# Rita-zi/WavTokenizer

Measured on AMD Instinct MI355X. Metric: audio-seconds/sec encode+decode, 24 kHz 3 s clips, higher is better.
Workload: dtype f32 (split-f16 x3 products)

## Files before the change

include/wavtokenizer_amd.h:

```cpp
#ifndef WAVTOKENIZER_AMD_H
#define WAVTOKENIZER_AMD_H

#include <stddef.h>
#include <stdint.h>

#ifdef __cplusplus
extern "C" {
#endif

typedef enum {
    WT_OK = 0,
    WT_ERR_INVALID = -1,
    WT_ERR_MISSING_TENSOR = -2,
    WT_ERR_SHAPE = -3,
    WT_ERR_HIP = -4,
    WT_ERR_NOT_INITED = -5,
    WT_ERR_RANGE = -6,
    WT_ERR_LSTM_SYNC = -7,
    WT_ERR_INDEX = -8
} wt_status;

enum wt_status_bits {
    WT_STATUS_BIT_LSTM = 1,
    WT_STATUS_BIT_RANGE = 2,
// ... 144 lines not shown
    const float* A2;
    const float* B;
    const float* bias;
    const float* R;
    const float* gamma;
    float* C;
    float* C2;
    uint32_t* status;
} wt_gemm_desc;
typedef struct {
    int32_t BM, BN, waves_m, waves_n, stages, ks, prod, staged, bias_cache, G, tiles;
} wt_launch_form;
size_t wt_gemm_probe_workspace_bytes(const wt_gemm_desc* d);
int wt_gemm_probe(const wt_gemm_desc* d, wt_launch_form* form, void* workspace, void* stream);

enum { WT_OP_GN_APPLY = 0, WT_OP_GN_STATS = 1, WT_OP_ROWNORM = 2, WT_OP_SOFTMAX = 3, WT_OP_ISTFT_OLA = 4, WT_OP_CONV_FIRST = 5,
       WT_OP_CONV_LAST = 6, WT_OP_TRANSPOSE = 7, WT_OP_CONVTR = 8, WT_OP_ROW_SUMSQ = 9, WT_OP_S32_AMAX = 10 };
enum { WT_OPK_GN_TILE = 1, WT_OPK_GN_CHUNK = 2, WT_OPK_GN_STATS = 3, WT_OPK_ROWNORM = 4, WT_OPK_DWCONV_LN = 5,
       WT_OPK_SOFTMAX_REG = 6, WT_OPK_SOFTMAX_RMW = 7, WT_OPK_ISTFT_OLA = 8, WT_OPK_CONV_FIRST = 9, WT_OPK_CONV_LAST32 = 10,
       WT_OPK_CONV_LAST = 11, WT_OPK_TRANSPOSE = 12, WT_OPK_CONVTR = 13, WT_OPK_ROW_SUMSQ = 14, WT_OPK_S32_AMAX = 15,
       WT_OPK_TRANSPOSE_MIXED = 16, WT_OPK_GN_MIXED = 17, WT_OPK_DWCONV_LN_MIXED = 18, WT_OPK_SOFTMAX_REG_MIXED = 19,
       WT_OPK_SOFTMAX_RMW_MIXED = 20, WT_OPK_ISTFT_OLA_MIXED = 21 };
typedef struct {
    int32_t size;
    int32_t op;
    int32_t B, L, C;
    int32_t groups, mode, flag, out_s32;
    int32_t ld, k, stride, Cout, n_fft, hop, Kq;
    float eps;
    int64_t n;
// ... 42 lines not shown
```

wavtokenizer_amd/_capi.py:

```python
from __future__ import annotations

import ctypes
import os
from ctypes import POINTER, c_char_p, c_float, c_int32, c_int64, c_size_t, c_void_p

_HERE = os.path.dirname(os.path.abspath(__file__))
LIB_PATH = os.environ.get("WAVTOK_HIP_LIB") or os.path.join(_HERE, "libwavtok_hip.so")

EXPORTS = [
    "wt_last_error", "wt_version", "wt_model_create", "wt_model_destroy", "wt_model_export_bytes", "wt_model_export", "wt_packed_info", "wt_packed_verify", "wt_packed_bytes",
    "wt_model_create_packed", "wt_model_hop", "wt_model_weight_bytes",
    "wt_plan_create", "wt_plan_create_ex", "wt_plan_range_sites", "wt_plan_range_report", "wt_model_persistent_lstm", "wt_device_info", "wt_plan_destroy", "wt_plan_workspace_bytes", "wt_plan_frames", "wt_plan_num_launches", "wt_plan_graph_replays",
    "wt_plan_find_buffer", "wt_plan_buffer_info", "wt_plan_buffer_name", "wt_plan_status", "wt_plan_num_steps", "wt_plan_step_name",
    "wt_plan_set_timing", "wt_plan_read_timing", "wt_model_split_ok", "wt_model_status", "wt_model_take_bad_codes", "wt_encode", "wt_codes_to_features",
    "wt_decode", "wt_seanet_decode", "wt_head", "wt_unit_run", "wt_sconv1d", "wt_linear", "wt_conv1d_s32", "wt_vq_workspace_bytes",
    "wt_vq_nearest", "wt_vq_nearest_f32", "wt_resblock", "wt_resblock_down", "wt_gemm_probe_workspace_bytes", "wt_gemm_probe", "wt_op_probe",
    "wt_resampler_create", "wt_resampler_destroy", "wt_resampler_out_length", "wt_convert_audio", "wt_pcm16",
    "wt_linear_overlap_add", "wt_encode_mixed", "wt_plan_min_clip_length", "wt_sconv_geometry", "wt_decode_mixed",
]

WT_PLAN_ENCODE, WT_PLAN_DECODE, WT_PLAN_SEANET_DECODER, WT_PLAN_HEAD, WT_PLAN_UNIT_LSTM = 0, 1, 2, 3, 4
WT_PLAN_DECODE_MIXED = 5
WT_PLAN_FLAG_KEEP_STAGES = 1
WT_PLAN_FLAG_FP32_GEMM = 2
WT_PLAN_FLAG_STEP_LSTM = 4
WT_PLAN_FLAG_GRAPH = 8
WT_PLAN_FLAG_UNFUSED = 16
WT_PLAN_FLAG_RANGE_REPORT = 32
WT_PLAN_FLAG_MIXED_LENGTH = 64
WT_SITE_ENCODER, WT_SITE_BB_EMBED, WT_SITE_RES0, WT_SITE_RES1, WT_SITE_ATTN, WT_SITE_RES2, WT_SITE_RES3 = 0, 1, 2, 3, 4, 5, 6
WT_SITE_CNX0, WT_SITE_HEAD, WT_SITE_SEANET_DECODER = 7, 40, 41
# ... 11 lines not shown


class WtTensor(ctypes.Structure):
    _fields_ = [("name", c_char_p), ("data", POINTER(c_float)), ("numel", c_int64)]


class WtGemmDesc(ctypes.Structure):
    _fields_ = ([("size", c_int32), ("engine", c_int32), ("epi", c_int32), ("out", c_int32), ("pro", c_int32), ("b_is_act", c_int32),
                 ("M", c_int32), ("N", c_int32), ("K", c_int32)]
                + [(n, c_int32) for n in ("T_in", "T_out", "Cin", "taps", "stride", "dil", "pad_left", "pad_mode", "Tp",
                                         "K1", "nz", "tap_pair", "head_kb")]
                + [("alpha", c_float)]
                + [(n, c_int64) for n in ("a_bstride", "a_rstride", "a2_bstride", "a2_rstride", "w_rstride", "c_rstride",
                                         "r_rstride", "zA", "zW", "zC")]
                + [(n, c_void_p) for n in ("A", "A2", "B", "bias", "R", "gamma", "C", "C2", "status")])


class WtLaunchForm(ctypes.Structure):
    _fields_ = [(n, c_int32) for n in ("BM", "BN", "waves_m", "waves_n", "stages", "ks", "prod", "staged", "bias_cache", "G", "tiles")]


WT_OP_GN_APPLY, WT_OP_GN_STATS, WT_OP_ROWNORM, WT_OP_SOFTMAX, WT_OP_ISTFT_OLA, WT_OP_CONV_FIRST = 0, 1, 2, 3, 4, 5
WT_OP_CONV_LAST, WT_OP_TRANSPOSE, WT_OP_CONVTR, WT_OP_ROW_SUMSQ, WT_OP_S32_AMAX = 6, 7, 8, 9, 10
WT_OPK_NAMES = {1: "gn_tile", 2: "gn_chunk", 3: "gn_stats", 4: "rownorm", 5: "dwconv_ln", 6: "softmax_reg", 7: "softmax_rmw",
                8: "istft_ola", 9: "conv_first", 10: "conv_last32", 11: "conv_last", 12: "transpose", 13: "convtr",
                14: "row_sumsq", 15: "s32_amax", 16: "transpose_mixed", 17: "gn_mixed", 18: "dwconv_ln_mixed",
                19: "softmax_reg_mixed", 20: "softmax_rmw_mixed", 21: "istft_ola_mixed"}


class WtOpDesc(ctypes.Structure):
# ... 86 lines not shown
    lib.wt_head.argtypes = [c_void_p, c_void_p, c_void_p, c_void_p, c_void_p]
    lib.wt_sconv1d.argtypes = [c_void_p, c_void_p, c_void_p, c_void_p, c_int32, c_int64, c_int32, c_int32, c_int32,
                               c_int32, c_int32, c_int32, c_void_p]
    lib.wt_linear.argtypes = [c_void_p, c_void_p, c_void_p, c_void_p, c_int64, c_int32, c_int32, c_int32, c_void_p, c_void_p]
    lib.wt_conv1d_s32.argtypes = [c_void_p, c_void_p, c_void_p, c_void_p, c_int32, c_int64, c_int32, c_int32, c_int32,
                                  c_int32, c_int32, c_void_p, c_void_p]
    lib.wt_vq_workspace_bytes.argtypes = [c_int64, c_int32, c_int32]
    lib.wt_vq_workspace_bytes.restype = c_size_t
    lib.wt_vq_nearest.argtypes = [c_void_p, c_void_p, c_int64, c_int32, c_int32, c_void_p, c_void_p, c_void_p]
    lib.wt_vq_nearest_f32.argtypes = [c_void_p, c_void_p, c_int64, c_int32, c_int32, c_void_p, c_void_p, c_void_p]
    lib.wt_resblock.argtypes = [c_void_p] * 11 + [c_int32, c_int64, c_int32, c_int32, c_int32, c_int32, c_void_p]
    lib.wt_resblock_down.argtypes = [c_void_p] * 12 + [c_int32, c_int64, c_int32, c_void_p]
    lib.wt_gemm_probe_workspace_bytes.argtypes = [POINTER(WtGemmDesc)]
    lib.wt_gemm_probe_workspace_bytes.restype = c_size_t
    lib.wt_gemm_probe.argtypes = [POINTER(WtGemmDesc), POINTER(WtLaunchForm), c_void_p, c_void_p]
    lib.wt_op_probe.argtypes = [POINTER(WtOpDesc), POINTER(WtOpForm), c_void_p]
    lib.wt_resampler_create.argtypes = [c_int32, c_int32, c_int32, POINTER(c_void_p)]
    lib.wt_resampler_destroy.argtypes = [c_void_p]
    lib.wt_resampler_destroy.restype = None
    lib.wt_resampler_out_length.argtypes = [c_void_p, c_int64]
    lib.wt_resampler_out_length.restype = c_int64
    lib.wt_convert_audio.argtypes = [c_void_p, c_void_p, c_int32, c_int32, c_int64, c_void_p, c_void_p]
    lib.wt_pcm16.argtypes = [c_void_p, c_int64, ctypes.c_float, c_int32, c_void_p, c_void_p, c_void_p]
    lib.wt_linear_overlap_add.argtypes = [c_void_p, c_void_p, c_int32, c_int64, c_int64, c_int64, c_int64, c_void_p, c_void_p]
    return lib


lib = _load()


# ... 5 lines not shown
```

wavtokenizer_amd/csrc/common.h:

```cpp
#pragma once
#include <hip/hip_runtime.h>
#include <stdint.h>
#include <stdio.h>
#include <stdlib.h>
#include <mutex>
#include <string>

namespace wt {

void set_error(const std::string& msg);

#define WT_HIP_CHECK(expr)                                                                      \
    do {                                                                                        \
        hipError_t _e = (expr);                                                                 \
        if (_e != hipSuccess) {                                                                 \
            ::wt::set_error(std::string(#expr) + ": " + hipGetErrorString(_e));                 \
            return -4;                                                                          \
        }                                                                                       \
    } while (0)

struct PerDeviceOnce {
    std::mutex mu;
    bool seen[64] = {};
    template <class F> int run(F&& f) {
// ... 178 lines not shown
    int stage_off = 0;
    int pc_off = 0;
    float acc_scale = 1.f;
    const float* acc_scale_dev = nullptr;
    unsigned* status = nullptr;
    unsigned long long* dbg_stamps = nullptr;
    LaunchForm* form = nullptr;
};

int gemm_vq_parts(int N);
int check_gemm(const GemmArgs& a, int pro, int epi);
int check_gemm16s(const GemmArgs& a, int epi, int out, const int* mix_geom = nullptr);
int launch_gemm(const GemmArgs& a, int pro, int epi, hipStream_t s);
int launch_gemm16s(const GemmArgs& a, int epi, int out, hipStream_t s, const int* mix_geom = nullptr);
int gemm16s_vq_parts(int N);
int launch_split_s32(const float* x, void* out, long n, hipStream_t s, const float* scale_dev = nullptr);
int launch_unsplit_s32(const void* s32, float* out, long n, float inv_scale, hipStream_t s);
int launch_pow2_scales(const float* a, long na, const float* b, long nb, unsigned* bits2, float* out3, hipStream_t s);

int launch_conv_first(const float* wav, const float* w , const float* bias, float* y, int B, long T,
                      int k, int Cout, hipStream_t s);
int launch_conv_last(const float* x , const float* w , const float* bias, float* y ,
                     int B, long T, int Cin, int k, int elu_in, hipStream_t s);
int launch_transpose(const float* in, float* out, int B, int R, int C, hipStream_t s, int out_s32 = 0, const int* lens = nullptr);
size_t gn_part_floats(int B, int L, int groups);
int launch_gn_stats(const float* x, const float* gamma, const float* beta, float* scale, float* shift, int B, int L,
                    int C, int groups, float eps, hipStream_t s, float* part = nullptr, const int* lens = nullptr);
int launch_gn_apply(const float* x, const float* gamma, const float* beta, float* scale, float* shift, float* y,
                    int swish, int B, int L, int C, int groups, float eps, hipStream_t s, int out_s32 = 0, float* part = nullptr,
                    const int* lens = nullptr);
// ... 93 lines not shown
```

wavtokenizer_amd/csrc/gemm16s.hip:

```cpp
#include "common.h"

#include <cmath>
#include <stdlib.h>
#include <type_traits>

namespace wt {

typedef float f32x4 __attribute__((ext_vector_type(4)));
typedef float f32x16 __attribute__((ext_vector_type(16)));
typedef _Float16 f16x8 __attribute__((ext_vector_type(8)));
typedef __attribute__((address_space(3))) void* lds_ptr_t;
static constexpr int SBK = 32;

__device__ __forceinline__ int xcd_remap_s(int orig, int nwg) {
    int q = nwg >> 3, r = nwg & 7;
    int xcd = orig & 7, idx = orig >> 3;
    int base = xcd < r ? xcd * (q + 1) : r * (q + 1) + (xcd - r) * q;
    return base + idx;
}
__device__ __forceinline__ float elu_s(float x) { return elu_med3(x); }
__device__ __forceinline__ float erf_s(float a) {
    const float t = fabsf(a), s = a * a;
    float r = fmaf(-1.72853470e-5f, t, 3.83197126e-4f);
    const float u = fmaf(-3.88396438e-3f, t, 2.42546219e-2f);
// ... 162 lines not shown
#endif
#define G16_NAME gemm16s_kernel
#define G16_PARAMS
#define G16_MIX 0
#include "gemm16s_kernel.inc"
#undef G16_NAME
#undef G16_PARAMS
#undef G16_MIX
#define G16_NAME gemm16s_mixed_kernel
#define G16_PARAMS , const int* __restrict__ mix_geom
#define G16_MIX 1
#include "gemm16s_kernel.inc"
#undef G16_NAME
#undef G16_PARAMS
#undef G16_MIX

__global__ __launch_bounds__(256) void split_s32_kernel(const float* __restrict__ x, _Float16* __restrict__ out, long n,
                                                        const float* __restrict__ scale, unsigned* status) {
    const float sc = scale ? scale[0] : 1.f;
    float amax = 0.f;
    for (long i = (long)blockIdx.x * blockDim.x + threadIdx.x; i < n; i += (long)gridDim.x * blockDim.x) {
        const float v = x[i] * sc;
        amax = amax1(amax, v);
        const _Float16 h = (_Float16)v;
        const long g = (i >> 5) * 64 + (i & 31);
        out[g] = h;
        out[g + 32] = (_Float16)((v - (float)h) * 2048.f);
    }
    range_report(status, amax);
}
// ... 281 lines not shown
    a.group_m = tiles_n192 > 8 ? 8 : 1;
    if (tiles_n192 >= 12 && tiles_n192 % 6 == 0 && a.nz == 1) { a.group_m = 5; a.group_n = 6; }
    if (const char* e = lab_env("WT_GEMM16S_GM")) { a.group_m = atoi(e) > 0 ? atoi(e) : a.group_m; a.group_n = 0; }
    if (const char* e = lab_env("WT_GEMM16S_GN")) a.group_n = atoi(e);
    if (mix_geom) {
#define WT_CASE16S(E, O) if (epi == E && out == O) return launch16s_mixed<E, O>(a, s, mix_geom);
        WT_GEMM16S_MIXED_PAIRS(WT_CASE16S)
#undef WT_CASE16S
    }
#define WT_CASE16S(E, O) if (epi == E && out == O) return launch16s_tiled<E, O>(a, s);
    WT_GEMM16S_PAIRS(WT_CASE16S)
#undef WT_CASE16S
    set_error("gemm16s: unsupported epilogue / output-format pair");
    return -1;
}
#endif

}
```

wavtokenizer_amd/csrc/plan.cpp:

```cpp
#include "model.h"

namespace wt {

static bool site_fp32(const wt_plan* P, int site) { return (P->fp32_sites >> site) & 1u; }
static bool plan_fp32(const wt_plan* P) {
    if ((P->flags & WT_PLAN_FLAG_FP32_GEMM) || !P->model->s32_ok) return true;
    if (P->whole_site == SITE_SEADEC && !P->model->sd_s32_ok) return true;
    return P->whole_site >= 0 && site_fp32(P, P->whole_site);
}
static bool plan_unfused(const wt_plan* P) { return P->flags & WT_PLAN_FLAG_UNFUSED; }
static bool plan_s32(const wt_plan* P) { return !plan_unfused(P) && !plan_fp32(P); }

static int gemm_auto(const wt_plan* P, const GemmArgs& a, int pro, int epi, hipStream_t s) {
    if (P->model->f32_stale.load()) if (int rc = ensure_f32_weights(P->model)) return rc;
    return launch_gemm(a, pro, epi, s);
}

static void set_s32(GemmArgs& a, const S32Copy& c) {
    a.W_hi = c.p; a.acc_scale = c.acc_scale; a.tap_pair = c.tap_pair ? 1 : 0;
}

static int gemm_s32(const GemmArgs& a, int epi, int out, hipStream_t s, const int* mix = nullptr) {
    if (!a.W_hi) { set_error("internal: no S32 copy of this weight"); return WT_ERR_INVALID; }
    return launch_gemm16s(a, epi, out, s, mix);
// ... 155 lines not shown
        if (int rc = launch_fill_u32(s, 0u, (st_numel * sizeof(float) + 15) / 16 * 16, c.stream)) return rc;
        LstmArgs la;
        la.f16x3 = plan_fp32(P) ? 0 : 1;
        la.xg0 = P->ptr(c, xg); la.W0 = la.f16x3 ? w.W0h : w.W0; la.W1 = la.f16x3 ? w.W1h : w.W1; la.b1 = w.b1;
        la.h0 = s; la.h1 = s + (size_t)2 * H * Bp; la.c0 = s + (size_t)4 * H * Bp; la.c1 = la.c0 + (size_t)B * H;
        la.x = P->ptr(c, xin); la.y = P->ptr(c, y); la.B = B; la.L = L; la.H = H; la.elu_out = elu_out ? 1 : 0;
        la.out_s32 = y_s32 ? 1 : 0;
        for (int t = 0; t <= L; ++t)
            if (int rc = launch_lstm_step(la, t, c.stream)) return rc;
        return 0;
    }, L + 2);
    return y;
}

static int plan_resblock_s32(wt_plan* P, const ConvW& c3, const ConvW& sc, const ConvW& cat, int B, long T, int x_raw,
                             int x_elu, const std::string& name, long x_off = 0, long x_bstride = 0, int mix_word = -1) {
    if (!cat.s32.p) { set_error("internal: unfused S32 resblock without an S32 shortcut + conv1 weight"); return -1; }
    const int C = sc.cout;
    const int h = P->buf(name + ".h", (size_t)B * T * (C / 2), BUF_S32 | BUF_ELU);
    GemmArgs a3 = sconv_args(c3, B, T, 1, 1);
    GemmBufs b3{x_elu, -1, h};
    b3.x_off = x_off; b3.mix_word = mix_word >= 0 ? mix_word + GEOM_C3 : -1;
    if (x_bstride) a3.a_bstride = x_bstride;
    gemm_step(P, true, a3, b3, PRO_NONE, EPI_BIAS_ELU, OUT_S32);
    const int o = P->buf(name, (size_t)B * T * C, BUF_S32 | BUF_ELU);
    GemmArgs ac = sconv_args(sc, B, T, 1, 1);
    ac.W = cat.w; ac.w_rstride = cat.cin; ac.bias = cat.b; ac.K = cat.cin; ac.Cin = cat.cin;
    set_s32(ac, cat.s32);
    ac.K1 = C; ac.a2_bstride = T * (C / 2); ac.a2_rstride = C / 2;
    if (x_bstride) ac.a_bstride = x_bstride;
    GemmBufs bc{x_raw, h, o};
    bc.x_off = x_off; bc.mix_word = mix_word >= 0 ? mix_word + GEOM_SC : -1;
    gemm_step(P, true, ac, bc, PRO_NONE, EPI_BIAS_ELU, OUT_S32);
// ... 76 lines not shown
                a.wav = c.in_f; a.e0_w = M->e0_w; a.e0_b = M->e0_b;
                a.W3 = st.c3.w; a.b3 = st.c3.b; a.W1 = st.c1.w; a.b1 = st.c1.b; a.Ws = st.sc.w; a.bs = st.sc.b;
                a.Wd = st.down.w; a.bd = st.down.b; a.y_down = P->ptr(c, y); a.R = st.r;
                a.B = B; a.T = (int)Tc; a.C = st.C;
                return launch_resblock16_down(a, c.stream, geom >= 0 ? &mix : nullptr);
            }, 1, "resblock.fused_down");
            x = y; Tc = ad.T_out; idx += 3;
            continue;
        }
        const std::string name = "enc." + std::to_string(idx);
        const int stage_word = GEOM_STAGE0 + (int)si * GEOM_STAGE_WORDS;
        if (r.fused)
            x = plan_resblock(P, st.c3, st.c1, st.sc, B, Tc, x, name, fuse_elu, (si == 0 && fold_e0) ? M : nullptr, 0, 0, r.s32,
                              mixed ? stage_word + GEOM_C3 : -1);
        else if (r.s32)
            x = plan_resblock_s32(P, st.c3, st.sc, st.cat, B, Tc, x, x_elu, name, 0, 0, mixed ? stage_word : -1);
        else
            x = plan_resblock(P, st.c3, st.c1, st.sc, B, Tc, x, name, fuse_elu);
        if (x < 0) return WT_ERR_INVALID;
        const bool next_s32 = !last && !route[si + 1].fused && route[si + 1].s32;
        const int y = P->buf(out, ynum, next_s32 ? BUF_S32 : BUF_F32);
        const int y2 = (next_s32 || (last && lstm_s32)) ? P->buf(out + ".s32", ynum, BUF_S32 | (next_s32 ? BUF_ELU : 0)) : -1;
        GemmBufs bd{x, -1, y, y2};
        bd.mix_word = mixed ? stage_word + GEOM_DOWN : -1;
        gemm_step(P, r.s32, ad, bd, fuse_elu ? PRO_NONE : PRO_ELU, EPI_BIAS,
                  next_s32 ? OUT_S32_DUAL_ELU : (y2 >= 0 ? OUT_F32_AND_S32 : OUT_F32));
        if (next_s32) x_elu = y2;
        if (last) x_s32 = y2;
        x = y; Tc = ad.T_out; idx += 3;
    }
    const int L = (int)Tc;
// ... 326 lines not shown
```

wavtokenizer_amd/csrc/probe.cpp:

```cpp
#include "model.h"

using namespace wt;

extern "C" {

int wt_codes_to_features(const wt_model* m, const int64_t* codes, int32_t K, int32_t B, int64_t L, float* features,
                         void* stream) {
    if (!m || !codes || !features) { set_error("wt_codes_to_features: null argument"); return WT_ERR_INVALID; }
    if (K < 1 || K > m->arch.num_quantizers) { set_error("wt_codes_to_features: K exceeds the number of codebooks"); return WT_ERR_INVALID; }
    DeviceGuard dg(m->device);
    if (!dg.ok) { set_error("hipSetDevice failed"); return WT_ERR_HIP; }
    return launch_codes_to_features(codes, m->embed.w, K, m->arch.vq_bins, B, L, 512, features, static_cast<hipStream_t>(stream),
                                    m->bad_codes_dev);
}

int wt_sconv1d(const float* x, const float* w, const float* bias, float* y, int32_t B, int64_t T, int32_t Cin,
               int32_t Cout, int32_t k, int32_t stride, int32_t dilation, int32_t elu_input, void* stream) {
    ConvW cw; cw.w = const_cast<float*>(w); cw.b = const_cast<float*>(bias); cw.cout = Cout; cw.cin = Cin; cw.k = k;
    GemmArgs a = sconv_args(cw, B, T, stride, dilation);
    a.A = x; a.C = y;
    return launch_gemm(a, elu_input ? PRO_ELU : PRO_NONE, EPI_BIAS, static_cast<hipStream_t>(stream));
}

static int split_pair(const float* w, long nw, const float* x, long nx, char* ws_w, char* ws_x, char* tail, GemmArgs& a,
// ... 79 lines not shown
    a.w_rstride = d->w_rstride; a.bias = d->bias; a.M = d->M; a.N = d->N; a.K = d->K;
    a.C = d->C; a.c_rstride = d->c_rstride; a.C2 = d->C2; a.R = d->R; a.r_rstride = d->r_rstride; a.gamma = d->gamma;
    a.alpha = d->alpha; a.nz = d->nz; a.zA = d->zA; a.zW = d->zW; a.zC = d->zC; a.head_kb = d->head_kb; a.tap_pair = d->tap_pair ? 1 : 0;
    if (d->engine == 1) {
        a.A = d->A; a.W = d->B;
        return check_gemm(a, d->pro, d->epi) ? WT_ERR_INVALID : WT_OK;
    }
    const ProbeLayout L = probe_layout(*d);
    a.A = reinterpret_cast<const float*>(ws);
    a.A2 = d->A2 ? reinterpret_cast<const float*>(ws + L.oA2) : nullptr;
    a.W = d->B; a.W_hi = ws + L.oB;
    a.status = reinterpret_cast<unsigned*>(d->status);
    return check_gemm16s(a, d->epi, d->out) ? WT_ERR_INVALID : WT_OK;
}

size_t wt_gemm_probe_workspace_bytes(const wt_gemm_desc* d) {
    if (!d || d->size != (int32_t)sizeof(wt_gemm_desc) || d->engine != 0 || d->M <= 0 || d->T_out <= 0 || d->nz < 1) return 0;
    return probe_layout(*d).total;
}

int wt_gemm_probe(const wt_gemm_desc* d, wt_launch_form* form, void* workspace, void* stream) {
    char* ws = static_cast<char*>(workspace);
    GemmArgs a;
    if (int rc = probe_args(d, ws, a)) return rc;
    hipStream_t s = static_cast<hipStream_t>(stream);
    LaunchForm lf;
    a.form = &lf;
    if (d->engine == 1) {
        if (int rc = launch_gemm(a, d->pro, d->epi, s)) return rc;
    } else {
        const ProbeLayout L = probe_layout(*d);
        float* scale_dev = reinterpret_cast<float*>(ws + L.oScale);
        float scale = 1.f;
        if (!d->b_is_act) {
            std::vector<float> h((size_t)L.nB);
            WT_HIP_CHECK(hipMemcpyAsync(h.data(), d->B, (size_t)L.nB * 4, hipMemcpyDeviceToHost, s));
            WT_HIP_CHECK(hipStreamSynchronize(s));
            float amax = 0.f;
            for (long z = 0; z < d->nz; ++z)
                for (long n = 0; n < d->N; ++n)
                    for (long k = 0; k < d->K; ++k) {
                        const float v = std::fabs(h[(size_t)(z * d->zW + n * d->w_rstride + k)]);
                        if (!(v <= 3.0e38f)) { set_error("wt_gemm_probe: a non-finite weight has no S32 copy"); return WT_ERR_INVALID; }
                        amax = std::max(amax, v);
                    }
            scale = s32_weight_scale(amax);
            uint32_t bits;
            memcpy(&bits, &scale, 4);
            if (int rc = launch_fill_u32(scale_dev, bits, 16, s)) return rc;
            a.acc_scale = 1.f / scale;
        }
        if (int rc = launch_split_s32(d->B, ws + L.oB, L.nB, s, scale != 1.f ? scale_dev : nullptr)) return rc;
        if (int rc = launch_split_s32(d->A, ws, L.nA, s)) return rc;
        if (d->A2) if (int rc = launch_split_s32(d->A2, ws + L.oA2, L.nA2, s)) return rc;
        if (int rc = launch_gemm16s(a, d->epi, d->out, s)) return rc;
    }
    if (form) *form = wt_launch_form{lf.BM, lf.BN, lf.waves_m, lf.waves_n, lf.stages, lf.ks, lf.prod, lf.staged, lf.bias_cache, lf.G, lf.tiles};
    return WT_OK;
}

static int op_probe_check(const wt_op_desc* d) {
    auto bad = [](const char* m) { set_error(std::string("wt_op_probe: ") + m); return (int)WT_ERR_INVALID; };
    if (!d || (d->size != (int32_t)sizeof(wt_op_desc) && d->size != (int32_t)offsetof(wt_op_desc, lengths))) return bad("descriptor missing or of another size");
    const int32_t* lengths = d->size == (int32_t)sizeof(wt_op_desc) ? d->lengths : nullptr;
    if (lengths) {
        if (reinterpret_cast<uintptr_t>(lengths) & 3) return bad("lengths misaligned");
        const bool aware = d->op == WT_OP_GN_APPLY || d->op == WT_OP_GN_STATS || (d->op == WT_OP_ROWNORM && d->mode == RN_DWCONV) ||
                           d->op == WT_OP_SOFTMAX || d->op == WT_OP_ISTFT_OLA || d->op == WT_OP_TRANSPOSE;
        if (!aware) return bad("this op has no length-aware launch");
        if (d->op == WT_OP_SOFTMAX && (d->L <= 0 || d->n % d->L)) return bad("the length-aware softmax needs whole clips of L rows");
    }
// ... 188 lines not shown
```

Measured before the change: 38630.

## Fuse resblock k3 conv, ELU and concatenated shortcut GEMM into one chained kernel

Adds a persistent chained GEMM kernel for the S32 resblock. It computes the 3-tap conv, applies bias and ELU, and splits the hidden activation into f16 hi/lo halves held in LDS. The same kernel then runs the concatenated 1x1 and shortcut GEMM, so the hidden tensor never makes a round trip through global memory and one launch is saved per resblock. The kernel holds more LDS and registers and is limited to C of 128 or 256; a probe API is also added for testing.

```diff
diff --git a/include/wavtokenizer_amd.h b/include/wavtokenizer_amd.h
--- a/include/wavtokenizer_amd.h
+++ b/include/wavtokenizer_amd.h
@@ -182,6 +182,22 @@
 size_t wt_gemm_probe_workspace_bytes(const wt_gemm_desc* d);
 int wt_gemm_probe(const wt_gemm_desc* d, wt_launch_form* form, void* workspace, void* stream);
 
+typedef struct {
+    int32_t size;
+    int32_t C, clips, T;
+    int64_t c_rstride;
+    const float* x_elu;
+    const float* x_raw;
+    const float* w3;
+    const float* b3;
+    const float* wcat;
+    const float* bcat;
+    float* out;
+    uint32_t* status;
+} wt_gemm_chain_desc;
+size_t wt_gemm_chain_probe_workspace_bytes(const wt_gemm_chain_desc* d);
+int wt_gemm_chain_probe(const wt_gemm_chain_desc* d, wt_launch_form* form, void* workspace, void* stream);
+
 enum { WT_OP_GN_APPLY = 0, WT_OP_GN_STATS = 1, WT_OP_ROWNORM = 2, WT_OP_SOFTMAX = 3, WT_OP_ISTFT_OLA = 4, WT_OP_CONV_FIRST = 5,
        WT_OP_CONV_LAST = 6, WT_OP_TRANSPOSE = 7, WT_OP_CONVTR = 8, WT_OP_ROW_SUMSQ = 9, WT_OP_S32_AMAX = 10 };
 enum { WT_OPK_GN_TILE = 1, WT_OPK_GN_CHUNK = 2, WT_OPK_GN_STATS = 3, WT_OPK_ROWNORM = 4, WT_OPK_DWCONV_LN = 5,
diff --git a/wavtokenizer_amd/_capi.py b/wavtokenizer_amd/_capi.py
--- a/wavtokenizer_amd/_capi.py
+++ b/wavtokenizer_amd/_capi.py
@@ -15,6 +15,7 @@
     "wt_plan_set_timing", "wt_plan_read_timing", "wt_model_split_ok", "wt_model_status", "wt_model_take_bad_codes", "wt_encode", "wt_codes_to_features",
     "wt_decode", "wt_seanet_decode", "wt_head", "wt_unit_run", "wt_sconv1d", "wt_linear", "wt_conv1d_s32", "wt_vq_workspace_bytes",
     "wt_vq_nearest", "wt_vq_nearest_f32", "wt_resblock", "wt_resblock_down", "wt_gemm_probe_workspace_bytes", "wt_gemm_probe", "wt_op_probe",
+    "wt_gemm_chain_probe_workspace_bytes", "wt_gemm_chain_probe",
     "wt_resampler_create", "wt_resampler_destroy", "wt_resampler_out_length", "wt_convert_audio", "wt_pcm16",
     "wt_linear_overlap_add", "wt_encode_mixed", "wt_plan_min_clip_length", "wt_sconv_geometry", "wt_decode_mixed",
 ]
@@ -56,6 +57,11 @@
                 + [(n, c_int64) for n in ("a_bstride", "a_rstride", "a2_bstride", "a2_rstride", "w_rstride", "c_rstride",
                                          "r_rstride", "zA", "zW", "zC")]
                 + [(n, c_void_p) for n in ("A", "A2", "B", "bias", "R", "gamma", "C", "C2", "status")])
+
+
+class WtGemmChainDesc(ctypes.Structure):
+    _fields_ = ([(n, c_int32) for n in ("size", "C", "clips", "T")] + [("c_rstride", c_int64)]
+                + [(n, c_void_p) for n in ("x_elu", "x_raw", "w3", "b3", "wcat", "bcat", "out", "status")])
 
 
 class WtLaunchForm(ctypes.Structure):
@@ -172,6 +178,9 @@
     lib.wt_gemm_probe_workspace_bytes.argtypes = [POINTER(WtGemmDesc)]
     lib.wt_gemm_probe_workspace_bytes.restype = c_size_t
     lib.wt_gemm_probe.argtypes = [POINTER(WtGemmDesc), POINTER(WtLaunchForm), c_void_p, c_void_p]
+    lib.wt_gemm_chain_probe_workspace_bytes.argtypes = [POINTER(WtGemmChainDesc)]
+    lib.wt_gemm_chain_probe_workspace_bytes.restype = c_size_t
+    lib.wt_gemm_chain_probe.argtypes = [POINTER(WtGemmChainDesc), POINTER(WtLaunchForm), c_void_p, c_void_p]
     lib.wt_op_probe.argtypes = [POINTER(WtOpDesc), POINTER(WtOpForm), c_void_p]
     lib.wt_resampler_create.argtypes = [c_int32, c_int32, c_int32, POINTER(c_void_p)]
     lib.wt_resampler_destroy.argtypes = [c_void_p]
diff --git a/wavtokenizer_amd/csrc/common.h b/wavtokenizer_amd/csrc/common.h
--- a/wavtokenizer_amd/csrc/common.h
+++ b/wavtokenizer_amd/csrc/common.h
@@ -216,6 +216,9 @@
 int launch_gemm(const GemmArgs& a, int pro, int epi, hipStream_t s);
 int launch_gemm16s(const GemmArgs& a, int epi, int out, hipStream_t s, const int* mix_geom = nullptr);
 int gemm16s_vq_parts(int N);
+bool gemm16s_chain_fits(int C);
+int check_gemm16s_chain(const GemmArgs& a3, const GemmArgs& ac);
+int launch_gemm16s_chain(const GemmArgs& a3, const GemmArgs& ac, hipStream_t s);
 int launch_split_s32(const float* x, void* out, long n, hipStream_t s, const float* scale_dev = nullptr);
 int launch_unsplit_s32(const void* s32, float* out, long n, float inv_scale, hipStream_t s);
 int launch_pow2_scales(const float* a, long na, const float* b, long nb, unsigned* bits2, float* out3, hipStream_t s);
diff --git a/wavtokenizer_amd/csrc/gemm16s.hip b/wavtokenizer_amd/csrc/gemm16s.hip
--- a/wavtokenizer_amd/csrc/gemm16s.hip
+++ b/wavtokenizer_amd/csrc/gemm16s.hip
@@ -200,6 +200,317 @@
 #undef G16_NAME
 #undef G16_PARAMS
 #undef G16_MIX
+
+struct ChainArgs {
+    const char* Xe;
+    const char* Xr;
+    long xe_bstride, xe_rstride, xr_bstride, xr_rstride;
+    const char* W3;
+    const char* Wc;
+    long w3_rstride, wc_rstride;
+    const float* b3;
+    const float* bc;
+    float s3, sc;
+    float* C;
+    long c_rstride;
+    int M, T, Tp, pad_left;
+    unsigned* status;
+    unsigned long long* stamp_start;
+    unsigned long long* stamp_end;
+    int res_off, tab_off, bias_off, stage_off;
+};
+
+template <int C, int BM, int WAVES_M, int WAVES_N>
+__global__ __launch_bounds__(64 * WAVES_M * WAVES_N) void gemm16s_chain_kernel(const ChainArgs p) {
+    constexpr int N1 = C / 2, NKC = C / 32, NK1 = 3 * NKC, NKH = N1 / 32, NPASS = C / 128, NK2 = NKC + NKH;
+    constexpr int NS = NK1 + NPASS * NK2;
+    constexpr int NW = WAVES_M * WAVES_N, NT = 64 * NW;
+    constexpr int WM = BM / WAVES_M, WN1 = N1 / WAVES_N, WN2 = 128 / WAVES_N;
+    constexpr int TNH1 = WN1 / 32, TNH2 = WN2 / 32;
+    constexpr int STG = (BM + 128) * 128;
+    constexpr int NPA = BM / 8 / NW, NPB = 128 / 8 / NW, NPT = NPA + NPB;
+    constexpr int NSTAGE = 3;
+    static_assert(NW == 8 && WM == 32 && WN1 == 32 && (WN2 == 32 || WN2 == 64) && (NPASS == 1 || NPASS == 2), "tile forms of C = 128 / 256");
+    static_assert((NKC & (NKC - 1)) == 0 && BM % 64 == 0, "K tiles per tap: a power of two");
+    extern __shared__ __attribute__((aligned(1024))) char smem_s[];
+    constexpr unsigned OOB = 0x80000000u;
+
+    const int tid = threadIdx.x, lane = tid & 63;
+    const int wave = __builtin_amdgcn_readfirstlane(tid >> 6);
+    const int wm = wave / WAVES_N, wn = wave % WAVES_N;
+    const int ntiles = (p.M + BM - 1) / BM, G = gridDim.x;
+    const int nclips = p.M / p.T;
+    if (p.stamp_start && tid == 0)
+        __hip_atomic_fetch_min(p.stamp_start, (unsigned long long)__builtin_amdgcn_s_memrealtime(), __ATOMIC_RELAXED, __HIP_MEMORY_SCOPE_AGENT);
+    auto first_clip = [&](int bm) { return (bm * BM < p.M ? bm * BM : p.M - 1) / p.T; };
+
+    char* const res = smem_s + p.res_off;
+    unsigned* const s_tab = reinterpret_cast<unsigned*>(smem_s + p.tab_off);
+    float* const s_bias = reinterpret_cast<float*>(smem_s + p.bias_off);
+    for (int e = tid; e < N1 + C; e += NT) s_bias[e] = e < N1 ? p.b3[e] : p.bc[e - N1];
+
+    auto build_table = [&](int vb, int par) {
+        if (vb >= ntiles) return;
+        const int bm = xcd_remap_s(vb, ntiles);
+        const int clip0 = first_clip(bm);
+        unsigned* tab = s_tab + par * 4 * BM;
+        for (int e = tid; e < 4 * BM; e += NT) {
+            const int tp = e / BM, r = e - tp * BM;
+            const int m = bm * BM + r;
+            unsigned off = OOB;
+            if (m < p.M) {
+                const int b = m / p.T;
+                const int t = m - b * p.T;
+                if (tp < 3) {
+                    int pos = t - p.pad_left + tp;
+                    pos = pos < 0 ? -pos : pos;
+                    pos = pos >= p.Tp ? 2 * (p.Tp - 1) - pos : pos;
+                    if (pos < p.T) off = (unsigned)(((long)(b - clip0) * p.xe_bstride + (long)pos * p.xe_rstride) * 4);
+                } else {
+                    off = (unsigned)(((long)(b - clip0) * p.xr_bstride + (long)t * p.xr_rstride) * 4);
+                }
+            }
+            tab[e] = off;
+        }
+    };
+
+    const int prow = lane >> 3;
+    int a_row[NPA];
+    unsigned a_chunk[NPA], a_voff[NPA], w3_voff[NPB], wc_voff[NPB];
+#pragma unroll
+    for (int i = 0; i < NPA; ++i) {
+        const int q = wave + NW * i;
+        a_row[i] = q * 8 + prow;
+        a_chunk[i] = (unsigned)(((lane & 7) ^ (((q & 1) << 2) | (lane >> 4))) * 16);
+    }
+#pragma unroll
+    for (int j = 0; j < NPB; ++j) {
+        const int q = BM / 8 + wave + NW * j;
+        const unsigned ch = (unsigned)(((lane & 7) ^ (((q & 1) << 2) | (lane >> 4))) * 16);
+        const int n = (wave + NW * j) * 8 + prow;
+        w3_voff[j] = n < N1 ? (unsigned)((long)n * p.w3_rstride * 4) + ch : OOB;
+        wc_voff[j] = (unsigned)((long)n * p.wc_rstride * 4) + ch;
+    }
+    auto rsrc = [](const char* base, long span) {
+        return __builtin_amdgcn_make_buffer_rsrc(const_cast<char*>(base), 0, (int)(span < 0x7fffffffL ? span : 0x7fffffffL), 0x00020000);
+    };
+    const __amdgpu_buffer_rsrc_t rsW3 = rsrc(p.W3, (long)N1 * p.w3_rstride * 4);
+    const __amdgpu_buffer_rsrc_t rsWc0 = rsrc(p.Wc, 128L * p.wc_rstride * 4);
+    const __amdgpu_buffer_rsrc_t rsWc1 = rsrc(p.Wc + (NPASS - 1) * 128L * p.wc_rstride * 4, 128L * p.wc_rstride * 4);
+    __amdgpu_buffer_rsrc_t rsXe, rsXr;
+    int l_vb = blockIdx.x, l_par = 0, l_step = 0;
+    unsigned l_mask = 0;
+    auto set_arow = [&](int trow) {
+        const unsigned* tab = s_tab + (l_par * 4 + trow) * BM;
+#pragma unroll
+        for (int i = 0; i < NPA; ++i) a_voff[i] = tab[a_row[i]] + a_chunk[i];
+    };
+    auto loader_set_tile = [&](int vb, int par) {
+        l_vb = vb; l_par = par; l_step = 0;
+        if (vb >= ntiles) { l_mask = OOB; return; }
+        const int clip0 = first_clip(xcd_remap_s(vb, ntiles));
+        rsXe = rsrc(p.Xe + (long)clip0 * p.xe_bstride * 4, ((long)(nclips - clip0 - 1) * p.xe_bstride + (long)p.T * p.xe_rstride) * 4);
+        rsXr = rsrc(p.Xr + (long)clip0 * p.xr_bstride * 4, ((long)(nclips - clip0 - 1) * p.xr_bstride + (long)p.T * p.xr_rstride) * 4);
+        set_arow(0);
+    };
+    auto load_tile = [&](int stage) {
+        char* sbase = smem_s + stage * STG + wave * 1024;
+        if (l_step < NK1) {
+            const int ci = l_step & (NKC - 1);
+#pragma unroll
+            for (int i = 0; i < NPA; ++i)
+                __builtin_amdgcn_raw_ptr_buffer_load_lds(rsXe, (lds_ptr_t)(sbase + NW * i * 1024), 16, (int)(a_voff[i] | l_mask), ci * 128, 0, 0);
+#pragma unroll
+            for (int j = 0; j < NPB; ++j)
+                __builtin_amdgcn_raw_ptr_buffer_load_lds(rsW3, (lds_ptr_t)(sbase + (BM / 8 + NW * j) * 1024), 16, (int)(w3_voff[j] | l_mask), l_step * 128, 0, 0);
+        } else {
+            const int u = l_step - NK1;
+            const bool pass1 = NPASS == 2 && u >= NK2;
+            const int v = pass1 ? u - NK2 : u;
+            const unsigned amask = v < NKC ? l_mask : OOB;
+#pragma unroll
+            for (int i = 0; i < NPA; ++i)
+                __builtin_amdgcn_raw_ptr_buffer_load_lds(rsXr, (lds_ptr_t)(sbase + NW * i * 1024), 16, (int)(a_voff[i] | amask), v * 128, 0, 0);
+            if (pass1) {
+#pragma unroll
+                for (int j = 0; j < NPB; ++j)
+                    __builtin_amdgcn_raw_ptr_buffer_load_lds(rsWc1, (lds_ptr_t)(sbase + (BM / 8 + NW * j) * 1024), 16, (int)(wc_voff[j] | l_mask), v * 128, 0, 0);
+            } else {
+#pragma unroll
+                for (int j = 0; j < NPB; ++j)
+                    __builtin_amdgcn_raw_ptr_buffer_load_lds(rsWc0, (lds_ptr_t)(sbase + (BM / 8 + NW * j) * 1024), 16, (int)(wc_voff[j] | l_mask), v * 128, 0, 0);
+            }
+        }
+        ++l_step;
+        if (l_step == NS) {
+            if (l_mask == 0) loader_set_tile(l_vb + G, l_par ^ 1);
+            else l_step = 0;
+        } else if (l_step < NK1) {
+            if ((l_step & (NKC - 1)) == 0) set_arow(l_step / NKC);
+        } else if (l_step == NK1) {
+            set_arow(3);
+        }
+    };
+
+    const int r16 = lane & 15, q4 = lane >> 4;
+    const int fo16h = r16 * 128 + ((q4 ^ ((r16 >> 1) & 7)) * 16), fo16l = r16 * 128 + (((4 + q4) ^ ((r16 >> 1) & 7)) * 16);
+    const int offA = wm * WM * 128, offB1 = (BM + wn * WN1) * 128, offB2 = (BM + wn * WN2) * 128;
+    f32x4 am[2][2 * TNH2], ac[2][2 * TNH2];
+    struct FragA { f16x8 h[2], l[2]; };
+    struct FragB { f16x8 h[TNH2], l[TNH2]; };
+    auto read_a = [&](const char* sA, FragA& F) {
+#pragma unroll
+        for (int i = 0; i < 2; ++i) {
+            F.h[i] = *reinterpret_cast<const f16x8*>(sA + i * 16 * 128 + fo16h);
+            F.l[i] = *reinterpret_cast<const f16x8*>(sA + i * 16 * 128 + fo16l);
+        }
+    };
+    auto read_b = [&](int stage, auto tnh_c, int half, int offB, FragB& F) {
+        constexpr int TNH = decltype(tnh_c)::value;
+        const char* sB = smem_s + stage * STG + offB + half * TNH * 16 * 128;
+#pragma unroll
+        for (int j = 0; j < TNH; ++j) {
+            F.h[j] = *reinterpret_cast<const f16x8*>(sB + j * 16 * 128 + fo16h);
+            F.l[j] = *reinterpret_cast<const f16x8*>(sB + j * 16 * 128 + fo16l);
+        }
+    };
+    auto mfma = [&](const FragA& A, const FragB& Bf, auto tnh_c, auto half_c) {
+        constexpr int TNH = decltype(tnh_c)::value, half = decltype(half_c)::value;
+#pragma unroll
+        for (int jj = 0; jj < TNH; ++jj)
+#pragma unroll
+            for (int i = 0; i < 2; ++i) {
+                constexpr int jbase = half * TNH;
+                f32x4& m = am[i][jbase + jj];
+                f32x4& c = ac[i][jbase + jj];
+                m = __builtin_amdgcn_mfma_f32_16x16x32_f16(Bf.h[jj], A.h[i], m, 0, 0, 0);
+                c = __builtin_amdgcn_mfma_f32_16x16x32_f16(Bf.l[jj], A.h[i], c, 0, 0, 0);
+                c = __builtin_amdgcn_mfma_f32_16x16x32_f16(Bf.h[jj], A.l[i], c, 0, 0, 0);
+            }
+    };
+    auto zero_acc = [&]() {
+#pragma unroll
+        for (int i = 0; i < 2; ++i)
+#pragma unroll
+            for (int j = 0; j < 2 * TNH2; ++j) { am[i][j] = (f32x4){0.f, 0.f, 0.f, 0.f}; ac[i][j] = (f32x4){0.f, 0.f, 0.f, 0.f}; }
+    };
+
+    float amax = 0.f;
+    const float lo_s3 = p.s3 * (1.f / 2048.f), lo_sc = p.sc * (1.f / 2048.f);
+    build_table(blockIdx.x, 0);
+    __syncthreads();
+    loader_set_tile(blockIdx.x, 0);
+    load_tile(0);
+    load_tile(1);
+    wait_vm_lgkm<NPT>();
+    __builtin_amdgcn_s_barrier();
+    FragA Fa;
+    FragB F0b, F1b;
+    int rs = 0, ws = NSTAGE - 1;
+    read_a(smem_s + offA, Fa);
+    read_b(0, std::integral_constant<int, TNH1>{}, 0, offB1, F0b);
+    auto kstep = [&](auto tc, auto tn, int offBc, int offBn, const char* a_next) {
+        load_tile(ws);
+        read_b(rs, tc, 1, offBc, F1b);
+        mfma(Fa, F0b, tc, std::integral_constant<int, 0>{});
+        wait_vm_lgkm<(NSTAGE - 2) * NPT>();
+        __builtin_amdgcn_s_barrier();
+        rs = rs + 1 == NSTAGE ? 0 : rs + 1;
+        ws = ws + 1 == NSTAGE ? 0 : ws + 1;
+        read_b(rs, tn, 0, offBn, F0b);
+        mfma(Fa, F1b, tc, std::integral_constant<int, 1>{});
+        read_a(a_next ? a_next : smem_s + rs * STG + offA, Fa);
+    };
+    constexpr std::integral_constant<int, TNH1> T1{};
+    constexpr std::integral_constant<int, TNH2> T2{};
+    float* __restrict__ Cg = p.C;
+    int c_par = 0;
+    for (int vb = blockIdx.x; vb < ntiles; vb += G, c_par ^= 1) {
+        build_table(vb + G, c_par ^ 1);
+        const int bm = xcd_remap_s(vb, ntiles);
+        const int m_w = bm * BM + wm * WM;
+        zero_acc();
+        for (int s = 0; s < NK1 - 1; ++s) kstep(T1, T1, offB1, offB1, nullptr);
+        kstep(T1, T2, offB1, offB2, nullptr);
+        {
+            char* rt = res + (wn * BM + wm * WM) * 128;
+#pragma unroll
+            for (int g = 0; g < 4; ++g) {
+                const int rw = 16 * (g >> 1) + r16, cw = 16 * (g & 1) + 4 * q4, sww = (rw >> 1) & 7;
+                const f32x4 m = am[g >> 1][g & 1], c = ac[g >> 1][g & 1];
+                f32x4 v;
+                v.x = fmaf(c.x, lo_s3, m.x * p.s3);
+                v.y = fmaf(c.y, lo_s3, m.y * p.s3);
+                v.z = fmaf(c.z, lo_s3, m.z * p.s3);
+                v.w = fmaf(c.w, lo_s3, m.w * p.s3);
+                v = v + *reinterpret_cast<const f32x4*>(s_bias + wn * WN1 + cw);
+                v.x = elu_s(v.x); v.y = elu_s(v.y); v.z = elu_s(v.z); v.w = elu_s(v.w);
+                amax = amax4(amax, v.x, v.y, v.z, v.w);
+                f16x4 hi, lo;
+                split4_f16(v.x, v.y, v.z, v.w, hi, lo);
+                if (m_w + rw >= p.M) { hi = (f16x4)(0); lo = (f16x4)(0); }
+                *reinterpret_cast<f16x4*>(rt + rw * 128 + (((cw >> 3) ^ sww) * 16) + 2 * (cw & 7)) = hi;
+                *reinterpret_cast<f16x4*>(rt + rw * 128 + (((4 + (cw >> 3)) ^ sww) * 16) + 2 * (cw & 7)) = lo;
+            }
+        }
+#pragma unroll
+        for (int pass = 0; pass < NPASS; ++pass) {
+            zero_acc();
+            for (int v = 0; v < NK2 - 1; ++v)
+                kstep(T2, T2, offB2, offB2, v + 1 >= NKC ? res + ((v + 1 - NKC) * BM + wm * WM) * 128 : nullptr);
+            if (pass + 1 < NPASS) kstep(T2, T2, offB2, offB2, nullptr);
+            else kstep(T2, T1, offB2, offB1, nullptr);
+            char* sc = smem_s + p.stage_off + wave * 4096;
+            const int n_w = pass * 128 + wn * WN2;
+#pragma unroll
+            for (int j = 0; j < WN2 / 32; ++j) {
+                const int n0 = n_w + j * 32;
+                f32x4 vb4[4];
+#pragma unroll
+                for (int g = 0; g < 4; ++g) {
+                    const f32x4 m = am[g >> 1][2 * j + (g & 1)], c = ac[g >> 1][2 * j + (g & 1)];
+                    f32x4 v;
+                    v.x = fmaf(c.x, lo_sc, m.x * p.sc);
+                    v.y = fmaf(c.y, lo_sc, m.y * p.sc);
+                    v.z = fmaf(c.z, lo_sc, m.z * p.sc);
+                    v.w = fmaf(c.w, lo_sc, m.w * p.sc);
+                    vb4[g] = v + *reinterpret_cast<const f32x4*>(s_bias + N1 + n0 + 16 * (g & 1) + 4 * q4);
+                }
+#pragma unroll
+                for (int g = 0; g < 4; ++g) {
+                    const int rw = 16 * (g >> 1) + r16, cw = 16 * (g & 1) + 4 * q4, sww = (rw >> 1) & 7;
+                    f32x4 v = vb4[g];
+                    v.x = elu_s(v.x); v.y = elu_s(v.y); v.z = elu_s(v.z); v.w = elu_s(v.w);
+                    amax = amax4(amax, v.x, v.y, v.z, v.w);
+                    f16x4 hi, lo;
+                    split4_f16(v.x, v.y, v.z, v.w, hi, lo);
+                    *reinterpret_cast<f16x4*>(sc + rw * 128 + (((cw >> 3) ^ sww) * 16) + 2 * (cw & 7)) = hi;
+                    *reinterpret_cast<f16x4*>(sc + rw * 128 + (((4 + (cw >> 3)) ^ sww) * 16) + 2 * (cw & 7)) = lo;
+                }
+                f32x4 q[4];
+#pragma unroll
+                for (int it = 0; it < 4; ++it) {
+                    const int r = 8 * it + (lane >> 3), ch = lane & 7;
+                    q[it] = *reinterpret_cast<const f32x4*>(sc + r * 128 + ((ch ^ ((r >> 1) & 7)) * 16));
+                }
+#pragma unroll
+                for (int it = 0; it < 4; ++it) {
+                    const int r = 8 * it + (lane >> 3), ch = lane & 7;
+                    const int m = m_w + r;
+                    if (m < p.M) store_c16<true>(Cg + (long)m * p.c_rstride + n0 + 4 * ch, q[it]);
+                }
+            }
+        }
+    }
+    range_report(p.status, amax);
+    if (p.stamp_end) {
+        wait_vm_lgkm<0>();
+        __syncthreads();
+        if (tid == 0)
+            __hip_atomic_fetch_max(p.stamp_end, (unsigned long long)__builtin_amdgcn_s_memrealtime(), __ATOMIC_RELAXED, __HIP_MEMORY_SCOPE_AGENT);
+    }
+    wait_vm_lgkm<0>();
+}
 
 __global__ __launch_bounds__(256) void split_s32_kernel(const float* __restrict__ x, _Float16* __restrict__ out, long n,
                                                         const float* __restrict__ scale, unsigned* status) {
@@ -511,6 +822,75 @@
     set_error("gemm16s: unsupported epilogue / output-format pair");
     return -1;
 }
+
+bool gemm16s_chain_fits(int C) { return C == 128 || C == 256; }
+
+int check_gemm16s_chain(const GemmArgs& a3, const GemmArgs& ac) {
+    GemmArgs t3 = a3, tc = ac;
+    t3.C = ac.C; tc.A2 = nullptr; tc.K1 = 0;
+    if (!ac.C || check_gemm16s(t3, EPI_BIAS_ELU, OUT_S32) || check_gemm16s(tc, EPI_BIAS_ELU, OUT_S32)) {
+        if (!ac.C) set_error("gemm16s chain: no output");
+        return -1;
+    }
+    const int C = ac.N;
+    if (!gemm16s_chain_fits(C) || a3.N != C / 2 || a3.Cin != C || a3.taps != 3 || a3.stride != 1 || a3.dil != 1 || a3.pad_mode != PAD_REFLECT ||
+        a3.tap_pair || a3.nz != 1 || ac.nz != 1 || ac.taps != 1 || ac.stride != 1 || ac.pad_left != 0 || ac.K != C + C / 2 || a3.M != ac.M ||
+        a3.T_out != ac.T_out || a3.T_in != a3.T_out || ac.T_in != ac.T_out || !a3.bias || !ac.bias || a3.acc_scale_dev || ac.acc_scale_dev) {
+        set_error("gemm16s chain: a k3 reflect conv C -> C/2 and a [x | h] contraction to C = 128 or 256 columns, both with a bias");
+        return -1;
+    }
+    return 0;
+}
+
+template <int C, int BM, int WMs, int WNs>
+static int launch_chain_one(const GemmArgs& a3, const GemmArgs& ac, hipStream_t s) {
+    static PerDeviceOnce attr_once;
+    constexpr size_t smem_cap = 160 * 1024;
+    constexpr size_t ring = 3ull * (BM + 128) * 128, resb = (size_t)BM * (C / 2) * 4, tabs = 2ull * 4 * BM * 4, biasb = (size_t)(C / 2 + C) * 4;
+    constexpr size_t scratch = (size_t)WMs * WNs * 4096;
+    constexpr bool alias = C / 128 == 1;
+    static_assert(!alias || scratch <= resb, "aliased scratch must fit the resident block");
+    constexpr size_t smem = ring + resb + tabs + biasb + (alias ? 0 : scratch);
+    static_assert(smem <= smem_cap, "LDS budget");
+    auto kern = gemm16s_chain_kernel<C, BM, WMs, WNs>;
+    if (int rc = attr_once.run([&]() -> int {
+        WT_HIP_CHECK(hipFuncSetAttribute(reinterpret_cast<const void*>(kern), hipFuncAttributeMaxDynamicSharedMemorySize, (int)smem));
+        return 0;
+    })) return rc;
+    ChainArgs p{};
+    p.Xe = reinterpret_cast<const char*>(a3.A); p.Xr = reinterpret_cast<const char*>(ac.A);
+    p.xe_bstride = a3.a_bstride; p.xe_rstride = a3.a_rstride; p.xr_bstride = ac.a_bstride; p.xr_rstride = ac.a_rstride;
+    p.W3 = static_cast<const char*>(a3.W_hi); p.Wc = static_cast<const char*>(ac.W_hi);
+    p.w3_rstride = a3.w_rstride; p.wc_rstride = ac.w_rstride;
+    p.b3 = a3.bias; p.bc = ac.bias; p.s3 = a3.acc_scale; p.sc = ac.acc_scale;
+    p.C = ac.C; p.c_rstride = ac.c_rstride;
+    p.M = ac.M; p.T = ac.T_out; p.Tp = a3.Tp; p.pad_left = a3.pad_left;
+    p.status = ac.status ? ac.status : g_launch.status;
+    if (g_launch.stamp_start && g_launch.stamp_end) {
+        p.stamp_start = g_launch.stamp_start; p.stamp_end = g_launch.stamp_end;
+        g_launch.stamp_used = true;
+    }
+    p.res_off = (int)ring; p.tab_off = (int)(ring + resb); p.bias_off = (int)(ring + resb + tabs);
+    p.stage_off = alias ? p.res_off : (int)(ring + resb + tabs + biasb);
+    const int ntiles = (ac.M + BM - 1) / BM;
+    int G = device_cus() & ~7;
+    if (G < 8 || ntiles <= G) G = ntiles;
+    else {
+        const int rounds = (ntiles + G - 1) / G;
+        const int g2 = (((ntiles + rounds - 1) / rounds) + 7) & ~7;
+        if (g2 < G) G = g2;
+    }
+    if (ac.form) *ac.form = LaunchForm{BM, 128, WMs, WNs, 3, 1, 0, 1, 1, G, ntiles};
+    hipLaunchKernelGGL(kern, dim3(G), dim3(64 * WMs * WNs), smem, s, p);
+    WT_HIP_CHECK(hipGetLastError());
+    return 0;
+}
+
+int launch_gemm16s_chain(const GemmArgs& a3, const GemmArgs& ac, hipStream_t s) {
+    if (int rc = check_gemm16s_chain(a3, ac)) return rc;
+    if (ac.N == 128) return launch_chain_one<128, 128, 4, 2>(a3, ac, s);
+    return launch_chain_one<256, 64, 2, 4>(a3, ac, s);
+}
 #endif
 
 }
diff --git a/wavtokenizer_amd/csrc/plan.cpp b/wavtokenizer_amd/csrc/plan.cpp
--- a/wavtokenizer_amd/csrc/plan.cpp
+++ b/wavtokenizer_amd/csrc/plan.cpp
@@ -193,9 +193,26 @@
 }
 
 static int plan_resblock_s32(wt_plan* P, const ConvW& c3, const ConvW& sc, const ConvW& cat, int B, long T, int x_raw,
-                             int x_elu, const std::string& name, long x_off = 0, long x_bstride = 0, int mix_word = -1) {
+                             int x_elu, const std::string& name, long x_off = 0, long x_bstride = 0, int mix_word = -1,
+                             bool chain = false) {
     if (!cat.s32.p) { set_error("internal: unfused S32 resblock without an S32 shortcut + conv1 weight"); return -1; }
     const int C = sc.cout;
+    const bool two_env = [] { const char* e = lab_env("WT_GEMM16S_NOCHAIN"); return e && e[0] == '1'; }();
+    if (chain && !two_env && mix_word < 0 && !(P->flags & WT_PLAN_FLAG_RANGE_REPORT) && gemm16s_chain_fits(C) && c3.s32.p &&
+        c3.k == 3 && c3.cout == C / 2 && x_off == 0 && x_bstride == 0) {
+        const int o = P->buf(name, (size_t)B * T * C, BUF_S32 | BUF_ELU);
+        GemmArgs a3 = sconv_args(c3, B, T, 1, 1);
+        GemmArgs ac = sconv_args(sc, B, T, 1, 1);
+        ac.W = cat.w; ac.w_rstride = cat.cin; ac.bias = cat.b; ac.K = cat.cin; ac.Cin = cat.cin;
+        set_s32(ac, cat.s32);
+        ac.K1 = C;
+        P->step({x_elu, x_raw, o}, [=](const RunCtx& c) {
+            GemmArgs g3 = a3, gc = ac;
+            g3.A = P->ptr(c, x_elu); gc.A = P->ptr(c, x_raw); gc.C = P->ptr(c, o);
+            return launch_gemm16s_chain(g3, gc, c.stream);
+        }, 1, name);
+        return o;
+    }
     const int h = P->buf(name + ".h", (size_t)B * T * (C / 2), BUF_S32 | BUF_ELU);
     GemmArgs a3 = sconv_args(c3, B, T, 1, 1);
     GemmBufs b3{x_elu, -1, h};
@@ -302,7 +319,7 @@
             x = plan_resblock(P, st.c3, st.c1, st.sc, B, Tc, x, name, fuse_elu, (si == 0 && fold_e0) ? M : nullptr, 0, 0, r.s32,
                               mixed ? stage_word + GEOM_C3 : -1);
         else if (r.s32)
-            x = plan_resblock_s32(P, st.c3, st.sc, st.cat, B, Tc, x, x_elu, name, 0, 0, mixed ? stage_word : -1);
+            x = plan_resblock_s32(P, st.c3, st.sc, st.cat, B, Tc, x, x_elu, name, 0, 0, mixed ? stage_word : -1, true);
         else
             x = plan_resblock(P, st.c3, st.c1, st.sc, B, Tc, x, name, fuse_elu);
         if (x < 0) return WT_ERR_INVALID;
diff --git a/wavtokenizer_amd/csrc/probe.cpp b/wavtokenizer_amd/csrc/probe.cpp
--- a/wavtokenizer_amd/csrc/probe.cpp
+++ b/wavtokenizer_amd/csrc/probe.cpp
@@ -117,6 +117,27 @@
     return check_gemm16s(a, d->epi, d->out) ? WT_ERR_INVALID : WT_OK;
 }
 
+static int split_weight(const float* B, long nB, long nz, long zW, long N, long w_rstride, long K, char* dst, float* scale_dev,
+                        float& acc_scale, hipStream_t s) {
+    std::vector<float> h((size_t)nB);
+    WT_HIP_CHECK(hipMemcpyAsync(h.data(), B, (size_t)nB * 4, hipMemcpyDeviceToHost, s));
+    WT_HIP_CHECK(hipStreamSynchronize(s));
+    float amax = 0.f;
+    for (long z = 0; z < nz; ++z)
+        for (long n = 0; n < N; ++n)
+            for (long k = 0; k < K; ++k) {
+                const float v = std::fabs(h[(size_t)(z * zW + n * w_rstride + k)]);
+                if (!(v <= 3.0e38f)) { set_error("wt_gemm_probe: a non-finite weight has no S32 copy"); return WT_ERR_INVALID; }
+                amax = std::max(amax, v);
+            }
+    const float scale = s32_weight_scale(amax);
+    uint32_t bits;
+    memcpy(&bits, &scale, 4);
+    if (int rc = launch_fill_u32(scale_dev, bits, 16, s)) return rc;
+    acc_scale = 1.f / scale;
+    return launch_split_s32(B, dst, nB, s, scale != 1.f ? scale_dev : nullptr);
+}
+
 size_t wt_gemm_probe_workspace_bytes(const wt_gemm_desc* d) {
     if (!d || d->size != (int32_t)sizeof(wt_gemm_desc) || d->engine != 0 || d->M <= 0 || d->T_out <= 0 || d->nz < 1) return 0;
     return probe_layout(*d).total;
@@ -134,30 +155,70 @@
     } else {
         const ProbeLayout L = probe_layout(*d);
         float* scale_dev = reinterpret_cast<float*>(ws + L.oScale);
-        float scale = 1.f;
-        if (!d->b_is_act) {
-            std::vector<float> h((size_t)L.nB);
-            WT_HIP_CHECK(hipMemcpyAsync(h.data(), d->B, (size_t)L.nB * 4, hipMemcpyDeviceToHost, s));
-            WT_HIP_CHECK(hipStreamSynchronize(s));
-            float amax = 0.f;
-            for (long z = 0; z < d->nz; ++z)
-                for (long n = 0; n < d->N; ++n)
-                    for (long k = 0; k < d->K; ++k) {
-                        const float v = std::fabs(h[(size_t)(z * d->zW + n * d->w_rstride + k)]);
-                        if (!(v <= 3.0e38f)) { set_error("wt_gemm_probe: a non-finite weight has no S32 copy"); return WT_ERR_INVALID; }
-                        amax = std::max(amax, v);
-                    }
-            scale = s32_weight_scale(amax);
-            uint32_t bits;
-            memcpy(&bits, &scale, 4);
-            if (int rc = launch_fill_u32(scale_dev, bits, 16, s)) return rc;
-            a.acc_scale = 1.f / scale;
+        if (d->b_is_act & 1) {
+            if (int rc = launch_split_s32(d->B, ws + L.oB, L.nB, s)) return rc;
+        } else if (int rc = split_weight(d->B, L.nB, d->nz, d->zW, d->N, d->w_rstride, d->K, ws + L.oB, scale_dev, a.acc_scale, s)) return rc;
+        if (int rc = launch_split_s32(d->A, ws, L.nA, s)) return rc;
+        if (d->A2) {
+            if (d->b_is_act & 2) WT_HIP_CHECK(hipMemcpyAsync(ws + L.oA2, d->A2, (size_t)L.nA2 * 4, hipMemcpyDeviceToDevice, s));
+            else if (int rc = launch_split_s32(d->A2, ws + L.oA2, L.nA2, s)) return rc;
         }
-        if (int rc = launch_split_s32(d->B, ws + L.oB, L.nB, s, scale != 1.f ? scale_dev : nullptr)) return rc;
-        if (int rc = launch_split_s32(d->A, ws, L.nA, s)) return rc;
-        if (d->A2) if (int rc = launch_split_s32(d->A2, ws + L.oA2, L.nA2, s)) return rc;
         if (int rc = launch_gemm16s(a, d->epi, d->out, s)) return rc;
     }
+    if (form) *form = wt_launch_form{lf.BM, lf.BN, lf.waves_m, lf.waves_n, lf.stages, lf.ks, lf.prod, lf.staged, lf.bias_cache, lf.G, lf.tiles};
+    return WT_OK;
+}
+
+struct ChainLayout { long nX = 0, nW3 = 0, nWc = 0; size_t oXr = 0, oW3 = 0, oWc = 0, oScale = 0, total = 0; };
+static ChainLayout chain_layout(const wt_gemm_chain_desc& d) {
+    ChainLayout L;
+    L.nX = (long)d.clips * d.T * d.C; L.nW3 = (long)(d.C / 2) * 3 * d.C; L.nWc = (long)d.C * (d.C + d.C / 2);
+    L.oXr = al256((size_t)L.nX * 4);
+    L.oW3 = L.oXr + al256((size_t)L.nX * 4);
+    L.oWc = L.oW3 + al256((size_t)L.nW3 * 4);
+    L.oScale = L.oWc + al256((size_t)L.nWc * 4);
+    L.total = L.oScale + 256;
+    return L;
+}
+static bool chain_desc_ok(const wt_gemm_chain_desc* d) {
+    return d && d->size == (int32_t)sizeof(wt_gemm_chain_desc) && d->C > 0 && d->C % 64 == 0 && d->C <= 4096 && d->clips > 0 && d->T > 0 &&
+           (long)d->clips * d->T < (long)INT_MAX / 2;
+}
+static int chain_args(const wt_gemm_chain_desc* d, char* ws, GemmArgs& a3, GemmArgs& ac) {
+    if (!chain_desc_ok(d)) { set_error("wt_gemm_chain_probe: descriptor missing, of another size, or bad extents"); return WT_ERR_INVALID; }
+    if (!d->x_elu || !d->x_raw || !d->w3 || !d->b3 || !d->wcat || !d->bcat || !d->out) { set_error("wt_gemm_chain_probe: null argument"); return WT_ERR_INVALID; }
+    if (!ws || (reinterpret_cast<uintptr_t>(ws) & 255)) { set_error("wt_gemm_chain_probe: needs a 256-byte aligned workspace"); return WT_ERR_INVALID; }
+    if (d->c_rstride < d->C) { set_error("wt_gemm_chain_probe: c_rstride < C"); return WT_ERR_INVALID; }
+    const ChainLayout L = chain_layout(*d);
+    const int C = d->C;
+    ConvW c3; c3.w = const_cast<float*>(d->w3); c3.b = const_cast<float*>(d->b3); c3.cout = C / 2; c3.cin = C; c3.k = 3;
+    ConvW sc; sc.w = const_cast<float*>(d->wcat); sc.b = const_cast<float*>(d->bcat); sc.cout = C; sc.cin = C; sc.k = 1;
+    a3 = sconv_args(c3, d->clips, d->T, 1, 1);
+    ac = sconv_args(sc, d->clips, d->T, 1, 1);
+    ac.w_rstride = C + C / 2; ac.K = C + C / 2; ac.Cin = C + C / 2; ac.K1 = C;
+    a3.A = reinterpret_cast<const float*>(ws); a3.W_hi = ws + L.oW3;
+    ac.A = reinterpret_cast<const float*>(ws + L.oXr); ac.W_hi = ws + L.oWc;
+    ac.C = d->out; ac.c_rstride = d->c_rstride;
+    ac.status = reinterpret_cast<unsigned*>(d->status);
+    return check_gemm16s_chain(a3, ac) ? WT_ERR_INVALID : WT_OK;
+}
+
+size_t wt_gemm_chain_probe_workspace_bytes(const wt_gemm_chain_desc* d) { return chain_desc_ok(d) ? chain_layout(*d).total : 0; }
+
+int wt_gemm_chain_probe(const wt_gemm_chain_desc* d, wt_launch_form* form, void* workspace, void* stream) {
+    char* ws = static_cast<char*>(workspace);
+    GemmArgs a3, ac;
+    if (int rc = chain_args(d, ws, a3, ac)) return rc;
+    hipStream_t s = static_cast<hipStream_t>(stream);
+    const ChainLayout L = chain_layout(*d);
+    float* scales = reinterpret_cast<float*>(ws + L.oScale);
+    if (int rc = split_weight(d->w3, L.nW3, 1, 0, d->C / 2, 3 * d->C, 3 * d->C, ws + L.oW3, scales, a3.acc_scale, s)) return rc;
+    if (int rc = split_weight(d->wcat, L.nWc, 1, 0, d->C, ac.K, ac.K, ws + L.oWc, scales + 4, ac.acc_scale, s)) return rc;
+    if (int rc = launch_split_s32(d->x_elu, ws, L.nX, s)) return rc;
+    if (int rc = launch_split_s32(d->x_raw, ws + L.oXr, L.nX, s)) return rc;
+    LaunchForm lf;
+    ac.form = &lf;
+    if (int rc = launch_gemm16s_chain(a3, ac, s)) return rc;
     if (form) *form = wt_launch_form{lf.BM, lf.BN, lf.waves_m, lf.waves_n, lf.stages, lf.ks, lf.prod, lf.staged, lf.bias_cache, lf.G, lf.tiles};
     return WT_OK;
 }
```

After: 38500. About the same (-0.3%).
